# NIFTy-PPL/NIFTy

Hardware: AMD Instinct MI355X
Metric: MGVI iters/sec on 1024^3 RGSpace CorrelatedField, 8 samples; achieved HBM GB/s (higher is better)
Workload: dtype f32

## Files before the change

include/niftyk.h:

```cpp
#ifndef NIFTYK_H
#define NIFTYK_H
#include <stddef.h>
#include <stdint.h>

#ifdef __cplusplus
extern "C" {
#endif

typedef enum {
  NK_OK = 0,
  NK_ERR_INVALID = -1,
  NK_ERR_UNSUPPORTED = -2,
  NK_ERR_RUNTIME = -3,
  NK_ERR_NOMEM = -4
} nk_status;

typedef enum { NK_F32 = 0, NK_F64 = 1 } nk_dtype;

#define NK_HARTLEY_NON_CANONICAL 0
#define NK_HARTLEY_CANONICAL 1

enum { NK_PRO_PLAIN = 0, NK_PRO_AMP = 1, NK_PRO_AMP_JVP = 2, NK_PRO_MUL = 3 };
enum { NK_EPI_AFFINE = 0, NK_EPI_MUL = 1, NK_EPI_VJP = 2, NK_EPI_LIKELIHOOD = 3, NK_EPI_NONLIN = 4 };
enum { NK_LH_GAUSS = 0, NK_LH_POISSON = 1 };
// ... 42 lines not shown
  int io32;
  const void* carry1;
  const void* carry2;
} nk_fuse;

typedef struct nk_plan nk_plan;

const char* nk_last_error(void);
int nk_version(void);

int nk_plan_create(nk_plan** plan, int ndim, const int64_t* shape, int dtype, int64_t batch);
int nk_plan_destroy(nk_plan* plan);
size_t nk_plan_workspace_bytes(const nk_plan* plan);
int nk_hartley(const nk_plan* plan, const void* in, void* out, double scale, int convention, void* workspace,
               void* stream);
int nk_hartley_fused(const nk_plan* plan, const nk_fuse* fuse, int convention, void* workspace, void* stream);
int nk_plan_route(const nk_plan* plan, int route[4]);
int nk_plan_pipe_ok(const nk_plan* plan, int chunks);
int nk_plan_sandwich(const nk_plan* plan);
int nk_hartley_sandwich(const nk_plan* plan, const nk_fuse* fuse, double scale_first, int convention, void* workspace,
                        void* stream);
int nk_hartley_sandwich_pair(const nk_plan* plan, const nk_fuse* fuse_a, const nk_fuse* fuse_b, double scale_first,
                             int convention, void* workspace_a, void* workspace_b, void* stream);
#define NK_MAX_GROUP 4
int nk_hartley_sandwich_group(const nk_plan* plan, const nk_fuse* fuses, int count, double scale_first, int convention,
                              void* const* workspaces, void* stream);
int nk_group_order(int64_t bid, int count, int64_t* member, int64_t* local);
int64_t nk_group_grid_size(int64_t per, int count);
int nk_fftn(const nk_plan* plan, const void* in, void* out, int inverse, double scale, void* workspace,
            void* stream);
int nk_plan_c2c_ok(const nk_plan* plan);
int nk_plan_c2c_lds(const nk_plan* plan, int64_t lds[3]);

int nk_profile_enable(int on);
int nk_profile_collect(double* ms, int64_t* count);

int nk_vdot(int64_t n, const void* a, const void* b, int dtype, double* result, int accumulate, void* stream);

int64_t nk_red_unit(int64_t n, int dtype);
int nk_red_layout(int64_t unit_elems, int k_local, int k_global, int seg_units, int seg_stride, int seg_off,
                  double* units_out);
int nk_red_finish(const double* units, int k_global, int nred, double* result, int accumulate, void* stream);
int nk_sum(int64_t n, const void* a, int dtype, double* result, int accumulate, void* stream);
int nk_stats(int64_t n, const void* a, int dtype, double* result3, void* stream);

enum { NK_OP_ADD = 0, NK_OP_SUB = 1, NK_OP_MUL = 2, NK_OP_DIV = 3 };
// ... 179 lines not shown
```

nifty_amd/_lib.py:

```python
import ctypes
import os

_HERE = os.path.dirname(os.path.abspath(__file__))
LIB_PATH = os.environ.get("NK_LIB_PATH") or os.path.join(_HERE, "csrc", "libniftyk.so")

NK_OK, NK_ERR_INVALID, NK_ERR_UNSUPPORTED, NK_ERR_RUNTIME, NK_ERR_NOMEM = 0, -1, -2, -3, -4
NK_F32, NK_F64 = 0, 1
PRO_PLAIN, PRO_AMP, PRO_AMP_JVP, PRO_MUL = 0, 1, 2, 3
EPI_AFFINE, EPI_MUL, EPI_VJP, EPI_LIKELIHOOD, EPI_NONLIN = 0, 1, 2, 3, 4
LH_GAUSS, LH_POISSON = 0, 1
NL_ID, NL_EXP, NL_SIGMOID = 0, 1, 2
OP_ADD, OP_SUB, OP_MUL, OP_DIV = 0, 1, 2, 3

_vp, _i, _i64, _d, _sz = ctypes.c_void_p, ctypes.c_int, ctypes.c_int64, ctypes.c_double, ctypes.c_size_t


class Fuse(ctypes.Structure):

    _fields_ = [
        ("pro", _i), ("in_", _vp), ("in2", _vp), ("pidx", _vp), ("amp", _vp), ("damp", _vp),
        ("epi", _i), ("out", _vp), ("scale", _d), ("offset", _d), ("mul", _vp), ("mul_scalar", _d),
        ("xi", _vp), ("addend", _vp), ("addend_scale", _d), ("accumulate", _i), ("abar", _vp), ("lh_kind", _i), ("nonlin", _i), ("data", _vp),
        ("icov", _vp), ("icov_scalar", _d), ("out2", _vp), ("value", _vp),
        ("afield", _vp), ("dampT", _vp), ("abar_copies", _i), ("abar_stride", _i64), ("dafield", _vp), ("w8", _vp),
# ... 22 lines not shown
                ("ntiles", _i32 * 3), ("reach", _i32 * 3), ("m", _i64), ("u", _vp), ("perm", _vp), ("bin_start", _vp),
                ("n_items", _i64), ("item", _vp), ("n_split", _i64), ("split_tile", _vp), ("split_slab", _vp), ("corr", _vp)]


class SamplePlan(ctypes.Structure):

    _fields_ = [("ndim", ctypes.c_int32), ("n", _i64 * 3), ("npoints", _i64), ("ncells", _i64), ("nlong", _i64), ("cell", _vp),
                ("frac", _vp), ("perm", _vp), ("cell_start", _vp), ("long_cell", _vp)]


SIGNATURES = {
    "nk_last_error": (ctypes.c_char_p, []),
    "nk_version": (_i, []),
    "nk_plan_create": (_i, [ctypes.POINTER(_vp), _i, ctypes.POINTER(_i64), _i, _i64]),
    "nk_plan_destroy": (_i, [_vp]),
    "nk_plan_workspace_bytes": (_sz, [_vp]),
    "nk_hartley": (_i, [_vp, _vp, _vp, _d, _i, _vp, _vp]),
    "nk_hartley_fused": (_i, [_vp, ctypes.POINTER(Fuse), _i, _vp, _vp]),
    "nk_plan_route": (_i, [_vp, ctypes.POINTER(_i)]),
    "nk_plan_sandwich": (_i, [_vp]),
    "nk_plan_pipe_ok": (_i, [_vp, _i]),
    "nk_hartley_sandwich": (_i, [_vp, ctypes.POINTER(Fuse), _d, _i, _vp, _vp]),
    "nk_hartley_sandwich_pair": (_i, [_vp, ctypes.POINTER(Fuse), ctypes.POINTER(Fuse), _d, _i, _vp, _vp, _vp]),
    "nk_hartley_sandwich_group": (_i, [_vp, ctypes.POINTER(Fuse), _i, _d, _i, _vp, _vp]),
    "nk_group_order": (_i, [_i64, _i, ctypes.POINTER(_i64), ctypes.POINTER(_i64)]),
    "nk_group_grid_size": (_i64, [_i64, _i]),
    "nk_fftn": (_i, [_vp, _vp, _vp, _i, _d, _vp, _vp]),
    "nk_plan_c2c_ok": (_i, [_vp]),
    "nk_plan_c2c_lds": (_i, [_vp, ctypes.POINTER(_i64)]),
    "nk_profile_enable": (_i, [_i]),
    "nk_profile_collect": (_i, [_vp, _vp]),
    "nk_vdot": (_i, [_i64, _vp, _vp, _i, _vp, _i, _vp]),
    "nk_product_field": (_i, [ctypes.POINTER(Product), _i, _vp, _i, _vp]),
    "nk_mirror_combine": (_i, [_i, ctypes.POINTER(_i64), ctypes.POINTER(_i), _i, ctypes.POINTER(_d), _vp, _vp, _d, _d, _i, _vp]),
    "nk_product_marginal_scratch": (_sz, [ctypes.POINTER(Product), _i]),
    "nk_product_marginal": (_i, [ctypes.POINTER(Product), _i, _vp, _vp, _vp, _vp]),
    "nk_red_unit": (_i64, [_i64, _i]),
    "nk_red_layout": (_i, [_i64, _i, _i, _i, _i, _i, _vp]),
    "nk_red_finish": (_i, [_vp, _i, _i, _vp, _i, _vp]),
    "nk_sum": (_i, [_i64, _vp, _i, _vp, _i, _vp]),
    "nk_stats": (_i, [_i64, _vp, _i, _vp, _vp]),
    "nk_binary": (_i, [_i, _i64, _vp, _d, _vp, _d, _vp, _i, _vp]),
    "nk_cplx_muldiv": (_i, [_i64, _vp, _i, _d, _d, _vp, _i, _d, _d, _i, _i, _vp, _i, _vp]),
    "nk_cplx_pointwise": (_i, [_i, _i64, _vp, _vp, _i, _vp]),
    "nk_axpby": (_i, [_i64, _d, _vp, _d, _vp, _vp, _i, _vp]),
    "nk_axpby_sqnorm": (_i, [_i64, _d, _vp, _d, _vp, _vp, _i, _vp, _i, _vp]),
# ... 108 lines not shown
```

nifty_amd/csrc/nk_fft.hip:

```cpp
#include <hip/hip_runtime.h>

#include <algorithm>

#include <cstdio>
#include <cstring>
#include <new>

#include "nk_fft_batch.h"

#include <mutex>
#include <vector>
using ProfScope = NkProfScope;
thread_local const NkBatchCtx* t_batch = nullptr;

template <typename T>
__device__ __forceinline__ void nk_run_stages(C2<T>* lds, int tid, int nthr, const NkLinePlan& lp, const NkTile& tl,
                                              const C2<T>* __restrict__ tw) {
  int L = lp.n;
  for (int s = 0; s < lp.nstage; ++s) {
    const int R = lp.radix[s];
    NK_STAGE_DISPATCH(R, lds, tid, nthr, lp, tl, L, tw, s)
    L /= R;
    __syncthreads();
  }
// ... 1088 lines not shown
  if (count == 1 || !nk_plan_batch_ok(P) || !nk_batch_class_ok(P->hp.g, fuse[0])) {
    for (int m = 0; m < count; ++m) {
      const int rc = P->hp.dtype == NK_F32 ? nk_run_hartley<float>(P, fuse[m], convention, workspace[m], st)
                                           : nk_run_hartley<double>(P, fuse[m], convention, workspace[m], st);
      if (rc != NK_OK) return rc;
    }
    return NK_OK;
  }
  if (P->hp.dtype == NK_F32) return nk_run_hartley_batch<float>(P, fuse, count, convention, workspace, st);
  return nk_run_hartley_batch<double>(P, fuse, count, convention, workspace, st);
}

static bool nk_strided_tile_divides(const nk_plan* P, int n, int64_t inner) {
  return P->hp.dtype == NK_F32 ? nk_fast_strided_ok<float>(n, inner) : nk_fast_strided_ok<double>(n, inner);
}
extern "C" int nk_plan_sandwich(const nk_plan* P) {
  if (!P || !nk_plan_uses_pipeline2(P) || !nk_fast_contig_ok(P->hp.g.h)) return 0;
  const NkGeom& g = P->hp.g;
  const int64_t rs = g.h + (P->hp.dtype == NK_F32 ? nk_pipe3_colpad<float>() : nk_pipe3_colpad<double>());
  if (g.ndim == 3 && !nk_strided_tile_divides(P, g.nm, rs)) return 0;
  return nk_strided_tile_divides(P, g.na, g.ndim == 3 ? (int64_t)g.nm * rs : rs) ? 1 : 0;
}

template <typename T>
static bool nk_contig3_quad_ok(int h) {
  return nk_with_fast_size(h, false, [](auto N) { return (bool)Contig3Tile<T, N()>::QUAD_OK; });
}
extern "C" int nk_plan_pipe_ok(const nk_plan* P, int chunks) {
  if (!nk_plan_sandwich(P) || chunks < 2 || (chunks & 1)) return 0;
  const NkGeom& g = P->hp.g;
  if (g.ndim != 3 || g.batch != 1 || g.na % chunks != 0) return 0;
  if (!nk_knobs().contig_quad || (nk_knobs().xmap & 4)) return 0;
  return (P->hp.dtype == NK_F32 ? nk_contig3_quad_ok<float>(g.h) : nk_contig3_quad_ok<double>(g.h)) ? 1 : 0;
}

template <typename T>
static int nk_run_sandwich(const nk_plan* P, const NkFuse& f, double scale_first, int convention, void* workspace, hipStream_t st,
                           bool with_final = true, NkPipe3* q_out = nullptr, bool with_first = true) {
  const NkHostPlan& hp = P->hp;
  const int sign = convention == NK_HARTLEY_CANONICAL ? -1 : 1;
  const int work_pad = nk_knobs().work_pad;
  const NkPipe3 q = nk_pipe3_setup<T>(hp, sign, work_pad, scale_first * (f.mul_scalar != 0.0 ? f.mul_scalar : 1.0));
  if (q_out) *q_out = q;
  if (nk_pipe3_work_elems(hp.g, nk_pipe3_colpad<T>(), work_pad) * sizeof(C2<T>) > hp.work_bytes)
    return nk_set_error(NK_ERR_RUNTIME, "nk_hartley_sandwich: plan workspace too small");
  if (128 * (q.ss > q.pm.s.inner ? q.ss : q.pm.s.inner) * (int64_t)sizeof(C2<T>) >= ((int64_t)1 << 32))
// ... 366 lines not shown
```

nifty_amd/csrc/nk_fft2.h:

```cpp
#pragma once
#include <type_traits>

#include "nk_fft_phases.h"

template <typename T>
struct TwConst {
  static NK_HD T c(int k) {
    constexpr double v[32] = {1.0,
                              0.99518472667219688624,
                              0.98078528040323044913,
                              0.95694033573220886494,
                              0.92387953251128675613,
                              0.88192126434835502971,
                              0.83146961230254523708,
                              0.77301045336273696081,
                              0.70710678118654752440,
                              0.63439328416364549822,
                              0.55557023301960222474,
                              0.47139673682599764856,
                              0.38268343236508977173,
                              0.29028467725446236764,
                              0.19509032201612826785,
                              0.09801714032956060199,
                              0.0,
// ... 196 lines not shown
#define NK_FINAL_LDS_KB 20
#endif
template <typename T, int NL, int EC = -1, int MINT = 1>
struct FinalTile {
  static constexpr int P = SchedF<T, NL>::P;
  static constexpr int PITCH = ContigLayout<NL, P>::PITCH;
  static constexpr int fit(int tile) {
    return (tile > MINT && (P * tile > 256 || 2 * tile * PITCH * (int)sizeof(T) > NK_FINAL_LDS_KB * 1024)) ? fit(tile / 2) : tile;
  }
  static constexpr int T0 = fit(16);
  static constexpr int TILE = (EC >= 0 && T0 / 2 >= MINT && P * (T0 / 2) >= 64) ? T0 / 2 : T0;
  static constexpr int THREADS = P * TILE;
  static constexpr int LDS_BYTES = 2 * TILE * PITCH * (int)sizeof(T);
};

#ifndef NK_FINAL_SINGLE_2D_KB
#define NK_FINAL_SINGLE_2D_KB 60
#endif
template <typename T, int NL>
constexpr bool nk_final_single_2d() {
  return FinalTile<T, NL, 2, 2>::LDS_BYTES > NK_FINAL_SINGLE_2D_KB * 1024;
}

#ifndef NK_NT_STORE
#define NK_NT_STORE 1
#endif
template <typename T>
NK_HD void nk_store_stream(C2<T>* p, C2<T> v) {
#if !defined(NK_HOST_EMU) && NK_NT_STORE
  typedef T __attribute__((ext_vector_type(2))) V2;
  V2 w;
  w.x = v.x, w.y = v.y;
  __builtin_nontemporal_store(w, reinterpret_cast<V2*>(p));
#else
  *p = v;
#endif
}

template <typename T>
NK_HD void nk_store_stream_s(T* p, T v) {
#if !defined(NK_HOST_EMU) && NK_NT_STORE
  __builtin_nontemporal_store(v, p);
#else
  *p = v;
#endif
}
// ... 508 lines not shown
  c.af = (const T*)f.afield;
  c.c1 = (const T*)f.carry1;
  c.c2 = (const T*)f.carry2;
  c.sc = (T)(f.scale * (EC == 1 ? f.mul_scalar : 1.0));
  c.off = (T)f.offset;
  c.asc = (T)f.addend_scale;
  c.accum = f.accumulate != 0;
  c.dot = EC == 2 && f.value != nullptr && f.addend != nullptr;
  c.keep = f.pipe_chunks < 0;
  c.stash = stash;
  return c;
}

#ifndef NK_FINAL_UNROLL
#define NK_FINAL_UNROLL 1
#endif
#ifndef NK_LH_UNROLL
#define NK_LH_UNROLL 4
#endif
template <typename T>
struct NkVjpOps {
  T x[4], d[4], o[4], p[4], q[4];
};
template <typename T, bool BOTH, int MODE, int STASH = 0>
NK_HD NkVjpOps<T> nk_final_vjp_load(const FinalCt<T>& c, int64_t ok, int64_t om, int k2, int k2m, const T* st = nullptr,
                                    int nkp = 0) {
  NkVjpOps<T> v;
  const bool add = MODE < 0 ? c.addend != nullptr : (MODE & 1) != 0;
  const bool run = MODE < 0 ? c.accum : (MODE & 2) != 0;
  const bool k1 = MODE < 0 ? c.c1 != nullptr : (MODE & 4) != 0;
  const bool k2nd = MODE < 0 ? c.c2 != nullptr : (MODE & 8) != 0;
  const int64_t rowb[4] = {ok, om, ok, om};
  const uint32_t colb[4] = {(uint32_t)k2, (uint32_t)k2m, (uint32_t)k2m, (uint32_t)k2};
#pragma unroll
  for (int i = 0; i < 4; ++i) {
    const bool on = BOTH || i < 2;
    if constexpr (STASH == 3)
      v.p[i] = on ? st[i * nkp] : (T)0;
    else
      v.p[i] = (on && k1) ? (c.c1 + rowb[i])[colb[i]] : (T)0;
    v.q[i] = (on && k2nd) ? (c.c2 + rowb[i])[colb[i]] : (T)0;
    if constexpr ((NK_NT_LOAD & 8) != 0) {
      v.x[i] = on ? nk_ld_stream((c.xi + rowb[i]) + colb[i]) : (T)0;
      v.d[i] = (on && add) ? nk_ld_stream((c.addend + rowb[i]) + colb[i]) : (T)0;
      if constexpr (STASH == 2)
        v.o[i] = on ? st[i * nkp] : (T)0;
      else
        v.o[i] = (on && run) ? nk_ld_stream((c.out + rowb[i]) + colb[i]) : (T)0;
    } else {
      v.x[i] = on ? (c.xi + rowb[i])[colb[i]] : (T)0;
      v.d[i] = (on && add) ? (c.addend + rowb[i])[colb[i]] : (T)0;
      if constexpr (STASH == 2)
        v.o[i] = on ? st[i * nkp] : (T)0;
      else
        v.o[i] = (on && run) ? (c.out + rowb[i])[colb[i]] : (T)0;
    }
  }
  return v;
}
template <typename T, bool BOTH, int MODE, int STASH = 0>
NK_HD double nk_final_vjp_apply(const FinalCt<T>& c, const NkVjpOps<T>& v, int64_t ok, int64_t om, bool self, T v0, T v1,
                                T v2, T v3, int k2, int k2m, T a, double& acc, T* st = nullptr, int nkp = 0) {
  const T t[4] = {v0 * c.sc, v1 * c.sc, v2 * c.sc, v3 * c.sc};
  const bool k1 = STASH == 3 || (MODE < 0 ? c.c1 != nullptr : (MODE & 4) != 0);
  const bool k2nd = MODE < 0 ? c.c2 != nullptr : (MODE & 8) != 0;
  T r[4];
#pragma unroll
  for (int i = 0; i < 4; ++i) {
    r[i] = nk_settle(a * t[i]);
    r[i] = nk_settle(nk_fma(c.asc, v.d[i], r[i]));
    if (k1) r[i] = v.p[i] + r[i];
    if (k2nd) r[i] = v.q[i] + r[i];
    r[i] = v.o[i] + r[i];
  }
  if (c.dot) {
    double e = (double)v.d[0] * (double)r[0];
    if (BOTH) e += (double)v.d[2] * (double)r[2];
    if (!self) e += (double)v.d[1] * (double)r[1] + (BOTH ? (double)v.d[3] * (double)r[3] : 0.0);
    acc += e;
  }
  T* outk = c.out + ok;
  T* outm = c.out + om;
  auto put = [&](T* p, T val, int image) {
    if constexpr (STASH == 1)
      st[image * nkp] = val;
    else if (c.keep)
      *p = val;
    else
      nk_store_stream_s(p, val);
  };
  put(outk + (uint32_t)k2, r[0], 0);
  if (BOTH) put(outk + (uint32_t)k2m, r[2], 2);
  double s = (double)v.x[0] * (double)t[0];
  if (BOTH) s += (double)v.x[2] * (double)t[2];
  if (!self) {
    put(outm + (uint32_t)k2m, r[1], 1);
    s += (double)v.x[1] * (double)t[1];
    if (BOTH) {
      put(outm + (uint32_t)k2, r[3], 3);
      s += (double)v.x[3] * (double)t[3];
    }
  }
  return s;
}

template <typename T, int EC, bool BOTH, int MODE = -1>
NK_HD double nk_final_slot(const NkFuse& f, const FinalCt<T>& c, int64_t ok, int64_t om, bool self, T sg, T fx, T fy, T gx,
// ... 29 lines not shown
      if (BOTH) nk_store_stream_s(outk + k2m, (T)(v2 * c.sc * m2));
      if (!self) {
        nk_store_stream_s(outm + k2m, (T)(v1 * c.sc * m1));
        if (BOTH) nk_store_stream_s(outm + k2, (T)(v3 * c.sc * m3));
      }
    } else {
      nk_store_stream_s(outk + k2, (T)(v0 * c.sc));
      if (BOTH) nk_store_stream_s(outk + k2m, (T)(v2 * c.sc));
      if (!self) {
        nk_store_stream_s(outm + k2m, (T)(v1 * c.sc));
        if (BOTH) nk_store_stream_s(outm + k2, (T)(v3 * c.sc));
      }
    }
    return 0.0;
  } else {
    static_assert(EC != 2, "the scatter epilogue runs through nk_final_vjp_load / nk_final_vjp_apply");
    return 0.0;
  }
}

template <typename T, int NL, int NH, bool BOTH, int MODE, int U, int STASH = 0>
NK_HD void nk_final_vjp_coeffs(const NkFuse& f, const FinalCt<T>& c, const FinalGroup<NH>& gp, const T* pre, const T* pim, T sg,
                               const int (&k2s)[U], int n_on, int hv, const T* afline, double* w8line, double& acc,
                               float& wmax) {
  constexpr int NKP = NL / 2 + 1;
  NkVjpOps<T> ops[U][NH];
  T a[U];
#pragma unroll
  for (int u = 0; u < U; ++u) {
    const int k2 = k2s[u], k2m = (NL - k2) & (NL - 1);
    a[u] = afline[k2];
#pragma unroll
    for (int h = 0; h < NH; ++h)
      if (MODE >= 0 || gp.mlo[h]) {
        if constexpr (STASH >= 2)
          ops[u][h] = nk_final_vjp_load<T, BOTH, MODE, STASH>(c, gp.okh[h], gp.omh[h], k2, k2m, c.stash + h * 4 * NKP + k2, NKP);
        else
          ops[u][h] = nk_final_vjp_load<T, BOTH, MODE>(c, gp.okh[h], gp.omh[h], k2, k2m);
      }
  }
#pragma unroll
  for (int u = 0; u < U; ++u) {
    if (u >= n_on) break;
    const int k2 = k2s[u], k2m = (NL - k2) & (NL - 1);
    const int d1 = k2 + (k2 >> 5), d2 = k2m + (k2m >> 5);
    double ssum = 0.0;
#pragma unroll
    for (int h = 0; h < NH; ++h) {
      if (MODE < 0 && !gp.mlo[h]) continue;
      const T fx = pre[gp.base[h] + d1], fy = pim[gp.base[h] + d1];
      const T gx = pre[gp.base[h] + d2], gy = pim[gp.base[h] + d2];
      if constexpr (STASH != 0)
        ssum += nk_final_vjp_apply<T, BOTH, MODE, STASH>(c, ops[u][h], gp.okh[h], gp.omh[h], gp.mlo[h] == 1, fx + sg * fy,
                                                         fx - sg * fy, gx + sg * gy, gx - sg * gy, k2, k2m, a[u], acc,
                                                         c.stash + h * 4 * NKP + k2, NKP);
      else
        ssum += nk_final_vjp_apply<T, BOTH, MODE>(c, ops[u][h], gp.okh[h], gp.omh[h], gp.mlo[h] == 1, fx + sg * fy, fx - sg * fy,
                                                  gx + sg * gy, gx - sg * gy, k2, k2m, a[u], acc);
    }
    if (w8line) {
      w8line[k2] = ssum;
      wmax = nk_wmax_join(wmax, nk_abs_up(ssum));
    } else {
      NK_VJP_SCATTER(f, f.pidx[gp.okh[hv] + k2], ssum);
    }
  }
}

template <typename T, int NL, int NH, bool BOTH, int MODE, int U, typename TD = T>
NK_HD void nk_final_lh_coeffs(const NkFuse& f, const FinalGroup<NH>& gp, const T* pre, const T* pim, T sg, const int (&k2s)[U],
                              int n_on, double& acc) {
  constexpr int MASK = BOTH ? 15 : 3;
  typename NkLhData<TD, MODE>::type d[U][NH][4];
#pragma unroll
  for (int u = 0; u < U; ++u) {
    const int k2 = k2s[u], k2m = (NL - k2) & (NL - 1);
#pragma unroll
    for (int h = 0; h < NH; ++h) {
// ... 3 lines not shown
  }
#pragma unroll
  for (int u = 0; u < U; ++u) {
    if (u >= n_on) break;
    const int k2 = k2s[u], k2m = (NL - k2) & (NL - 1);
    const int d1 = k2 + (k2 >> 5), d2 = k2m + (k2m >> 5);
    double ssum = 0.0;
#pragma unroll
    for (int h = 0; h < NH; ++h) {
      const T fx = pre[gp.base[h] + d1], fy = pim[gp.base[h] + d1];
      const T gx = pre[gp.base[h] + d2], gy = pim[gp.base[h] + d2];
      const int64_t o4[4] = {gp.okh[h] + k2, gp.omh[h] + k2m, gp.okh[h] + k2m, gp.omh[h] + k2};
      const T v4[4] = {fx + sg * fy, fx - sg * fy, gx + sg * gy, gx - sg * gy};
      double e = 0.0;
      nk_lh4_apply<T, MODE, MASK, TD>(f, o4, v4, d[u][h], e);
      ssum += e;
    }
    acc += ssum;
  }
}

template <typename T, int NL, int NH, int EC, bool BOTH, int MODE = -1, int STASH = 0>
NK_HD void nk_final_coeff(const NkFuse& f, const FinalCt<T>& c, const FinalGroup<NH>& gp, const T* pre, const T* pim, T sg,
                          int k2, int hv, const T* afline, double* w8line, double& acc, float& wmax) {
  if constexpr (EC == 2) {
    const int one[1] = {k2};
    nk_final_vjp_coeffs<T, NL, NH, BOTH, MODE, 1, STASH>(f, c, gp, pre, pim, sg, one, 1, hv, afline, w8line, acc, wmax);
  } else {
    const int k2m = (NL - k2) & (NL - 1);
    const int d1 = k2 + (k2 >> 5), d2 = k2m + (k2m >> 5);
    double ssum = 0.0;
#pragma unroll
    for (int h = 0; h < NH; ++h) {
      if (MODE <= 0 && !gp.mlo[h]) continue;
      const T fx = pre[gp.base[h] + d1], fy = pim[gp.base[h] + d1];
      const T gx = pre[gp.base[h] + d2], gy = pim[gp.base[h] + d2];
      ssum += nk_final_slot<T, EC, BOTH, MODE>(f, c, gp.okh[h], gp.omh[h], gp.mlo[h] == 1, sg, fx, fy, gx, gy, k2, k2m, (T)0,
                                               acc);
    }
    if constexpr (nk_ec_lh<EC>()) acc += ssum;
  }
}

struct NkPassF {
  NkGeom g;
  int A, M;
  int tiles_per_a;
  int blo;
  int64_t ss;
  int64_t rs;
// ... 153 lines not shown
    const int lane = tid - u * tps;
    constexpr int NH = COUPLES ? 2 : 1;
    FinalGroup<NH> gp;
    int any = 0;
    double* w8line = nullptr;
    const int b0g = couples ? bt0 * (TILE / 2) + u : bt0 * TILE + u;
    if (f.w8 && f.epi == NK_EPI_VJP)
      w8line = f.w8 + ((bat * (A / 2 + 1) + a) * (int64_t)(M / 2 + 1) + b0g) * (NL / 2 + 1);
#pragma unroll
    for (int h = 0; h < NH; ++h) {
      const int t = couples ? 2 * u + h : u;
      int b, bm;
      bool active, self;
      line_of(t, b, bm, active, self);
      if (h == 1 && !couples) active = false;
      gp.okh[h] = (((bat * A + a) * M + b)) * (int64_t)NL;
      gp.omh[h] = (((bat * A + am) * M + bm)) * (int64_t)NL;
      gp.base[h] = LY::addr(t, 0);
      gp.mlo[h] = active ? (self ? 1 : 3) : 0;
      any |= gp.mlo[h];
    }
    if constexpr (EC >= 0) {
      if (any) {
        const FinalCt<T> c = nk_final_ct<T, EC>(f, STASH != 0 ? stash + u * (NH * 4 * (NL / 2 + 1)) : nullptr);
        int hv = 0;
#pragma unroll
        for (int h = NH - 1; h >= 0; --h)
          if (gp.mlo[h]) hv = h;
        const T* afline = nullptr;
        if constexpr (EC == 2)
          afline = f.field_octant ? c.af + ((int64_t)a * (M / 2 + 1) + b0g) * (NL / 2 + 1) : c.af + gp.okh[hv];
        auto coefficients = [&](auto mode_c) {
          constexpr int MODE = decltype(mode_c)::value;
          if (lane < 2)
            nk_final_coeff<T, NL, NH, EC, false, MODE, STASH>(f, c, gp, pre, pim, sg, lane ? NL / 2 : 0, hv, afline, w8line, acc, wmax);
          if constexpr (nk_ec_lh<EC>() && MODE > 0) {
            constexpr int U = sizeof(T) == 8 ? (NK_LH_UNROLL + 1) / 2 : NK_LH_UNROLL;
            for (int k2 = 1 + lane; k2 < NL / 2; k2 += U * tps) {
              int ks[U], n_on = 0;
#pragma unroll
              for (int u = 0; u < U; ++u) {
                const int k = k2 + u * tps;
                const bool on = k < NL / 2;
                ks[u] = on ? k : k2;
                n_on += on;
              }
              nk_final_lh_coeffs<T, NL, NH, true, MODE, U, typename NkLhIo<T, EC>::type>(f, gp, pre, pim, sg, ks, n_on, acc);
            }
          } else if constexpr (EC == 2 && MODE >= 0 && NK_FINAL_UNROLL > 1) {
            constexpr int U = NK_FINAL_UNROLL;
            for (int k2 = 1 + lane; k2 < NL / 2; k2 += U * tps) {
              int ks[U], n_on = 0;
#pragma unroll
              for (int u = 0; u < U; ++u) {
                const int k = k2 + u * tps;
                const bool on = k < NL / 2;
                ks[u] = on ? k : k2;
                n_on += on;
              }
              nk_final_vjp_coeffs<T, NL, NH, true, MODE, U, STASH>(f, c, gp, pre, pim, sg, ks, n_on, hv, afline, w8line, acc, wmax);
            }
          } else {
            for (int k2 = 1 + lane; k2 < NL / 2; k2 += tps)
              nk_final_coeff<T, NL, NH, EC, true, MODE, STASH>(f, c, gp, pre, pim, sg, k2, hv, afline, w8line, acc, wmax);
          }
        };
        if constexpr (EC == 2) {
          bool full = true;
#pragma unroll
          for (int h = 0; h < NH; ++h) full = full && gp.mlo[h] != 0;
          switch (full ? (c.addend ? 1 : 0) | (c.accum ? 2 : 0) | (c.c1 ? 4 : 0) | (c.c2 ? 8 : 0) : -1) {
            case 0: coefficients(std::integral_constant<int, 0>{}); break;
            case 1: coefficients(std::integral_constant<int, 1>{}); break;
            case 2: coefficients(std::integral_constant<int, 2>{}); break;
            case 3: coefficients(std::integral_constant<int, 3>{}); break;
            case 6: coefficients(std::integral_constant<int, 6>{}); break;
            case 14: coefficients(std::integral_constant<int, 14>{}); break;
            default: coefficients(std::integral_constant<int, -1>{}); break;
          }
        } else if constexpr (nk_ec_lh<EC>()) {
          bool regular = true;
#pragma unroll
          for (int h = 0; h < NH; ++h) regular = regular && gp.mlo[h] == 3;
          const bool gauss = f.lh_kind == NK_LH_GAUSS;
          switch (regular && !(gauss && f.icov) ? (gauss ? 1 : 2) : -1) {
            case 1: coefficients(std::integral_constant<int, 1>{}); break;
            case 2: coefficients(std::integral_constant<int, 2>{}); break;
            default: coefficients(std::integral_constant<int, -1>{}); break;
          }
        } else {
          coefficients(std::integral_constant<int, -1>{});
        }
      }
    } else if (any) {
// ... 152 lines not shown
```

nifty_amd/csrc/nk_fft_batch.h:

```cpp
#pragma once
#include "nk_plan.h"
#include "nk_fft2.h"
#include "nk_util.h"

#ifndef NK_S0_WAVES
#define NK_S0_WAVES 1
#endif
#ifndef NK_PAIR_HAND_LDS_KB
#define NK_PAIR_HAND_LDS_KB 64
#endif
#ifndef NK_S1_TWO_WG
#define NK_S1_TWO_WG 0
#endif

template <typename T, bool COUPLES, int EC, int THREADS>
constexpr int nk_final_waves() {
  return THREADS > 256 ? 1 : (sizeof(T) == 8 && (COUPLES || EC == 2)) ? 2 : ((!COUPLES && sizeof(T) == 4 && (EC == 0 || EC == 1)) ? 4 : 3);
}

__device__ __forceinline__ void nk_flush_energy(const NkFuse& f, double acc, void* lds_raw) {
  if ((f.epi != NK_EPI_LIKELIHOOD && f.epi != NK_EPI_VJP) || f.value == nullptr) return;
  for (int off = 32; off > 0; off >>= 1) acc += __shfl_down(acc, off, 64);
  const int lane = threadIdx.x & 63, wave = threadIdx.x >> 6;
  const int nw = (blockDim.x + 63) >> 6;
// ... 52 lines not shown
static bool nk_batch_class_ok(const NkGeom& g, const nk_fuse& f) {
  if (nk_knobs().ec_generic || g.na < 512 || g.nl < 512) return false;
  const bool pro_ok = f.pro == NK_PRO_PLAIN || f.pro == NK_PRO_MUL ||
                      (f.field_octant && !f.io32 && (f.pro == NK_PRO_AMP || f.pro == NK_PRO_AMP_JVP));
  const bool epi_ok = f.epi == NK_EPI_MUL || (f.epi == NK_EPI_LIKELIHOOD && !f.io32) || f.epi == NK_EPI_NONLIN ||
                      (f.epi == NK_EPI_VJP && f.afield);
  return pro_ok && epi_ok;
}


template <typename T, int N, int PC>
int nk_twin_launch_strided(const NkPassS& ps, int64_t blocks, const C2<T>* tw, int xmap, hipStream_t st);
template <typename T, int NL, bool COUPLES, int EC>
int nk_twin_launch_final(const NkPassF& pf, int64_t blocks, const C2<T>* tw, int xmap, hipStream_t st);

template <typename T>
int nk_tl_first_axis(const NkPassS& s1, int n1, int n2, const NkFuse& f, const C2<T>* tw_n1, const C2<T>* tw_n2, const C2<T>* tw_full,
                     C2<T>* work, hipStream_t st);

template <typename T, int NL>
int nk_launch_final_pair(NkPassF pf, const NkFuse& fa, const NkFuse& fb, const C2<T>* tw, const C2<T>* worka, const C2<T>* workb,
                         hipStream_t st);

NK_HD void nk_group_decode(int64_t bid, int count, int64_t& member, int64_t& local) {
  const int64_t span = 8 * (int64_t)count;
  const int64_t g = bid / span, w = bid % span;
  member = w / 8;
  local = 8 * g + w % 8;
}
static inline int64_t nk_group_grid(int64_t per, int count) { return (per + 7) / 8 * 8 * count; }
struct NkGroupFuse {
  NkFuse f[NK_MAX_GROUP];
};
struct NkGroupWork {
  void* work[NK_MAX_GROUP];
};

#ifndef NK_QUAD_MAXW_F64_5
#define NK_QUAD_MAXW_F64_5 4
#endif
#ifndef NK_QUAD_MAXW_F64_8
#define NK_QUAD_MAXW_F64_8 8
#endif
#ifndef NK_QUAD_MAXW_F32_5
#define NK_QUAD_MAXW_F32_5 8
#endif
// ... 18 lines not shown
```

nifty_amd/csrc/nk_fft_p.hip:

```cpp
#include <hip/hip_runtime.h>

#include "nk_fft_batch.h"

#ifndef NK_PAIR_HAND_BUILD
#define NK_PAIR_HAND_BUILD 0
#endif
template <typename T, int NL>
struct PairTile {
  using CT = FinalTile<T, NL, 2, 2>;
  static constexpr int STASH_BYTES = CT::TILE * 4 * (NL / 2 + 1) * (int)sizeof(T);
  static constexpr int LDS_HAND = CT::LDS_BYTES + STASH_BYTES;
  static constexpr bool HAND_OK = NK_PAIR_HAND_BUILD != 0 && LDS_HAND <= NK_PAIR_HAND_LDS_KB * 1024;
};

#ifndef NK_PAIR_HAND_WAVES
#define NK_PAIR_HAND_WAVES 3
#endif
template <typename T, int NL, int HAND>
__global__ void __launch_bounds__((FinalTile<T, NL, 2, 2>::THREADS),
                                  (HAND ? (FinalTile<T, NL, 2, 2>::THREADS > 256 ? 1 : NK_PAIR_HAND_WAVES)
                                        : nk_final_waves<T, true, 2, FinalTile<T, NL, 2, 2>::THREADS>()))
    k2_final2(NkPassF p, NkFuse fa, NkFuse fb, const C2<T>* __restrict__ tw, const C2<T>* __restrict__ worka,
              const C2<T>* __restrict__ workb) {
  extern __shared__ __align__(16) unsigned char smem[];
  using CT = FinalTile<T, NL, 2, 2>;
  DeviceExec<T, SchedF<T, NL>::E> ex;
  const int64_t blk = (int64_t)blockIdx.x;
  T* stash = HAND ? (T*)(smem + CT::LDS_BYTES) : nullptr;
  fa.pipe_chunks = -1;
  {
    double acc = 0.0;
    float wmax = 0.0f;
    nk_final_body<T, NL, CT::TILE, true, 2, 1, HAND ? 1 : 0>(ex, p, fa, blk, (T*)smem, tw, worka, &acc, &wmax, stash);
    nk_flush_energy(fa, acc, smem);
    nk_flush_wmax(fa, wmax);
  }
  __syncthreads();
  {
    double acc = 0.0;
    float wmax = 0.0f;
    nk_final_body<T, NL, CT::TILE, true, 2, 1, HAND>(ex, p, fb, blk, (T*)smem, tw, workb, &acc, &wmax, stash);
    nk_flush_energy(fb, acc, smem);
    nk_flush_wmax(fb, wmax);
  }
}

template <typename T, int NL, int HAND>
static int nk_launch_final_pair_h(NkPassF pf, const NkFuse& fa, const NkFuse& fb, const C2<T>* tw, const C2<T>* worka,
                                  const C2<T>* workb, hipStream_t st) {
  using CT = FinalTile<T, NL, 2, 2>;
  const int LDS = HAND ? PairTile<T, NL>::LDS_HAND : CT::LDS_BYTES + nk_knobs().pair_pad_lds;
  pf.tiles_per_a = (pf.A > 1 && CT::TILE >= 2) ? (pf.M / 2 + 1 + CT::TILE / 2 - 1) / (CT::TILE / 2) : (pf.M + CT::TILE - 1) / CT::TILE;
  pf.blk0 = 0;
  const int64_t blocks = (int64_t)pf.g.batch * (pf.A / 2 + 1) * pf.tiles_per_a;
  const int64_t waves = blocks * ((CT::THREADS + 63) / 64);
  if ((fa.value_slots > 0 && waves > fa.value_slots) || (fb.value_slots > 0 && waves > fb.value_slots))
    return nk_set_error(NK_ERR_RUNTIME, "final pass: more wavefronts than reduction slots (nk_value_slot_count)");
  return nk_launch<k2_final2<T, NL, HAND>>("k2_final2", dim3((unsigned)blocks), dim3(CT::THREADS), LDS, st, pf, fa, fb, tw, worka, workb);
}

template <typename T, int NL>
int nk_launch_final_pair(NkPassF pf, const NkFuse& fa, const NkFuse& fb, const C2<T>* tw, const C2<T>* worka, const C2<T>* workb,
                         hipStream_t st) {
  if constexpr (PairTile<T, NL>::HAND_OK) {
    if (nk_knobs().pair_hand && pf.A > 1) {
      if (fa.out == fb.out && fb.accumulate) return nk_launch_final_pair_h<T, NL, 2>(pf, fa, fb, tw, worka, workb, st);
      if (fb.carry1 == fa.out && fb.out != fa.out) return nk_launch_final_pair_h<T, NL, 3>(pf, fa, fb, tw, worka, workb, st);
    }
  }
  return nk_launch_final_pair_h<T, NL, 0>(pf, fa, fb, tw, worka, workb, st);
}

#define NK_CASE(NN)                                                                                                             \
  template int nk_launch_final_pair<float, NN>(NkPassF, const NkFuse&, const NkFuse&, const C2<float>*, const C2<float>*,        \
                                               const C2<float>*, hipStream_t);                                                  \
  template int nk_launch_final_pair<double, NN>(NkPassF, const NkFuse&, const NkFuse&, const C2<double>*, const C2<double>*,     \
                                                const C2<double>*, hipStream_t);
NK_FAST_SIZES(NK_CASE)
#undef NK_CASE
```

nifty_amd/csrc/nk_plan.h:

```cpp
#pragma once
#include <cmath>
#include <cstdlib>
#include <vector>

#include "nk_fft_phases.h"

static inline NkLinePlan nk_make_line_plan(int n) {
  NkLinePlan lp{};
  lp.n = n;
  lp.nstage = 0;
  int rem = n;
  while (rem > 1) {
    int R;
    if (rem % 8 == 0) R = (rem == 16) ? 4 : 8;
    else if (rem % 4 == 0) R = 4;
    else if (rem % 2 == 0) R = 2;
    else if (rem % 3 == 0) R = 3;
    else if (rem % 5 == 0) R = 5;
    else if (rem % 7 == 0) R = 7;
    else {
      lp.nstage = -1;
      return lp;
    }
    if (lp.nstage == NK_MAX_STAGES) {
// ... 3 lines not shown
    lp.radix[lp.nstage++] = R;
    rem /= R;
  }
  int span = n;
  for (int s = 0; s < lp.nstage; ++s) {
    span /= lp.radix[s];
    lp.span[s] = span;
    lp.dradix[s] = nk_make_div(lp.radix[s]);
    lp.dspan[s] = nk_make_div(span);
    lp.dnbf[s] = nk_make_div(n / lp.radix[s]);
  }
  return lp;
}
static inline bool nk_factorable(int64_t n) { return n >= 1 && n < ((int64_t)1 << 30) && nk_make_line_plan((int)n).nstage >= 0; }

static inline int nk_env_int(const char* name, int dflt) {
  const char* v = getenv(name);
  return v ? atoi(v) : dflt;
}

#ifndef NK_XMAP_DEFAULT
#define NK_XMAP_DEFAULT 9
#endif
struct NkKnobs {
  int fast = 1;
  int pipeline = 2;
  int xmap = NK_XMAP_DEFAULT;
  int work_blo = 0;
  int work_pad = 2080;
  int contig_quad = 1;
  int ec_generic = 0;
  int two_level = 1;
  int skip_final = 0;
  int mid_wg_per_cu = 0;
  int pair_hand = 0;
  int pair_pad_lds = 0;
  int group = 1;
  int tile_divides = 0;
};
static inline NkKnobs nk_read_knobs() {
  NkKnobs k;
  k.fast = nk_env_int("NK_FAST", k.fast);
  k.pipeline = nk_env_int("NK_PIPELINE", k.pipeline);
  k.xmap = nk_env_int("NK_XMAP", k.xmap);
  k.work_blo = nk_env_int("NK_WORK_BLO", k.work_blo);
  k.work_pad = nk_env_int("NK_WORK_PAD", k.work_pad);
  k.contig_quad = nk_env_int("NK_CONTIG_QUAD", k.contig_quad);
  k.ec_generic = nk_env_int("NK_EC_GENERIC", k.ec_generic);
  k.two_level = nk_env_int("NK_TWO_LEVEL", k.two_level);
  k.skip_final = nk_env_int("NK_SKIP_FINAL", k.skip_final);
  k.mid_wg_per_cu = nk_env_int("NK_MID_WG_PER_CU", k.mid_wg_per_cu);
  k.pair_hand = nk_env_int("NK_PAIR_HAND", k.pair_hand);
  k.pair_pad_lds = nk_env_int("NK_PAIR_PAD_LDS", k.pair_pad_lds);
  k.group = nk_env_int("NK_GROUP", k.group);
  k.tile_divides = nk_env_int("NK_TILE_DIVIDES", k.tile_divides);
  return k;
}
inline NkKnobs nk_knobs() {
// ... 172 lines not shown
```

Before: 0.2199.

## Hand over paired final-pass VJP values through registers instead of LDS stash

Adds a register-resident hand-over (HAND bit 4) to the paired final Hartley kernel, so the first fused epilogue stashes its per-coefficient outputs in a per-thread register array that the second epilogue reads back directly. This avoids both re-reading the output/carry arrays from HBM and allocating an LDS stash. It is enabled by default through a new pair_hand default of 2. The cost is higher register pressure in the kernel, which may reduce occupancy or cause spills, and it relies on each thread visiting the same coefficients in both halves.

```diff
diff --git a/include/niftyk.h b/include/niftyk.h
--- a/include/niftyk.h
+++ b/include/niftyk.h
@@ -88,6 +88,7 @@
                         void* stream);
 int nk_hartley_sandwich_pair(const nk_plan* plan, const nk_fuse* fuse_a, const nk_fuse* fuse_b, double scale_first,
                              int convention, void* workspace_a, void* workspace_b, void* stream);
+int nk_plan_pair_hand(const nk_plan* plan);
 #define NK_MAX_GROUP 4
 int nk_hartley_sandwich_group(const nk_plan* plan, const nk_fuse* fuses, int count, double scale_first, int convention,
                               void* const* workspaces, void* stream);
diff --git a/nifty_amd/_lib.py b/nifty_amd/_lib.py
--- a/nifty_amd/_lib.py
+++ b/nifty_amd/_lib.py
@@ -68,6 +68,7 @@
     "nk_plan_pipe_ok": (_i, [_vp, _i]),
     "nk_hartley_sandwich": (_i, [_vp, ctypes.POINTER(Fuse), _d, _i, _vp, _vp]),
     "nk_hartley_sandwich_pair": (_i, [_vp, ctypes.POINTER(Fuse), ctypes.POINTER(Fuse), _d, _i, _vp, _vp, _vp]),
+    "nk_plan_pair_hand": (_i, [_vp]),
     "nk_hartley_sandwich_group": (_i, [_vp, ctypes.POINTER(Fuse), _i, _d, _i, _vp, _vp]),
     "nk_group_order": (_i, [_i64, _i, ctypes.POINTER(_i64), ctypes.POINTER(_i64)]),
     "nk_group_grid_size": (_i64, [_i64, _i]),
diff --git a/nifty_amd/csrc/nk_fft.hip b/nifty_amd/csrc/nk_fft.hip
--- a/nifty_amd/csrc/nk_fft.hip
+++ b/nifty_amd/csrc/nk_fft.hip
@@ -1134,6 +1134,13 @@
   return nk_strided_tile_divides(P, g.na, g.ndim == 3 ? (int64_t)g.nm * rs : rs) ? 1 : 0;
 }
 
+extern "C" int nk_plan_pair_hand(const nk_plan* P) {
+  if (!nk_plan_sandwich(P) || P->hp.g.ndim != 3) return -1;
+  const int nl = P->hp.g.nl;
+  if (P->hp.dtype == NK_F32) return nk_with_fast_size(nl, -1, [](auto N) { return nk_pair_hand_form<float, N()>(); });
+  return nk_with_fast_size(nl, -1, [](auto N) { return nk_pair_hand_form<double, N()>(); });
+}
+
 template <typename T>
 static bool nk_contig3_quad_ok(int h) {
   return nk_with_fast_size(h, false, [](auto N) { return (bool)Contig3Tile<T, N()>::QUAD_OK; });
diff --git a/nifty_amd/csrc/nk_fft2.h b/nifty_amd/csrc/nk_fft2.h
--- a/nifty_amd/csrc/nk_fft2.h
+++ b/nifty_amd/csrc/nk_fft2.h
@@ -242,6 +242,22 @@
   return FinalTile<T, NL, 2, 2>::LDS_BYTES > NK_FINAL_SINGLE_2D_KB * 1024;
 }
 
+template <typename T, int NL>
+struct FinalHand {
+  static constexpr int TPS = 2 * SchedF<T, NL>::P;
+  static constexpr int TRIPS = (NL / 2 - 1 + TPS - 1) / TPS;
+  static constexpr int N = (TRIPS + 1) * 2 * 4;
+};
+template <typename T, int NL>
+NK_HD T* nk_hand_of(T* hand, int tid) {
+#ifdef NK_HOST_EMU
+  return hand + (size_t)tid * FinalHand<T, NL>::N;
+#else
+  (void)tid;
+  return hand;
+#endif
+}
+
 #ifndef NK_NT_STORE
 #define NK_NT_STORE 1
 #endif
@@ -796,20 +812,24 @@
 struct NkVjpOps {
   T x[4], d[4], o[4], p[4], q[4];
 };
+template <int STASH>
+constexpr bool nk_stash_no_carry() {
+  return STASH == 5;
+}
 template <typename T, bool BOTH, int MODE, int STASH = 0>
 NK_HD NkVjpOps<T> nk_final_vjp_load(const FinalCt<T>& c, int64_t ok, int64_t om, int k2, int k2m, const T* st = nullptr,
                                     int nkp = 0) {
   NkVjpOps<T> v;
   const bool add = MODE < 0 ? c.addend != nullptr : (MODE & 1) != 0;
   const bool run = MODE < 0 ? c.accum : (MODE & 2) != 0;
-  const bool k1 = MODE < 0 ? c.c1 != nullptr : (MODE & 4) != 0;
-  const bool k2nd = MODE < 0 ? c.c2 != nullptr : (MODE & 8) != 0;
+  const bool k1 = !nk_stash_no_carry<STASH>() && (MODE < 0 ? c.c1 != nullptr : (MODE & 4) != 0);
+  const bool k2nd = !nk_stash_no_carry<STASH>() && (MODE < 0 ? c.c2 != nullptr : (MODE & 8) != 0);
   const int64_t rowb[4] = {ok, om, ok, om};
   const uint32_t colb[4] = {(uint32_t)k2, (uint32_t)k2m, (uint32_t)k2m, (uint32_t)k2};
 #pragma unroll
   for (int i = 0; i < 4; ++i) {
     const bool on = BOTH || i < 2;
-    if constexpr (STASH == 3)
+    if constexpr ((STASH & 3) == 3)
       v.p[i] = on ? st[i * nkp] : (T)0;
     else
       v.p[i] = (on && k1) ? (c.c1 + rowb[i])[colb[i]] : (T)0;
@@ -817,14 +837,14 @@
     if constexpr ((NK_NT_LOAD & 8) != 0) {
       v.x[i] = on ? nk_ld_stream((c.xi + rowb[i]) + colb[i]) : (T)0;
       v.d[i] = (on && add) ? nk_ld_stream((c.addend + rowb[i]) + colb[i]) : (T)0;
-      if constexpr (STASH == 2)
+      if constexpr ((STASH & 3) == 2)
         v.o[i] = on ? st[i * nkp] : (T)0;
       else
         v.o[i] = (on && run) ? nk_ld_stream((c.out + rowb[i]) + colb[i]) : (T)0;
     } else {
       v.x[i] = on ? (c.xi + rowb[i])[colb[i]] : (T)0;
       v.d[i] = (on && add) ? (c.addend + rowb[i])[colb[i]] : (T)0;
-      if constexpr (STASH == 2)
+      if constexpr ((STASH & 3) == 2)
         v.o[i] = on ? st[i * nkp] : (T)0;
       else
         v.o[i] = (on && run) ? (c.out + rowb[i])[colb[i]] : (T)0;
@@ -836,8 +856,8 @@
 NK_HD double nk_final_vjp_apply(const FinalCt<T>& c, const NkVjpOps<T>& v, int64_t ok, int64_t om, bool self, T v0, T v1,
                                 T v2, T v3, int k2, int k2m, T a, double& acc, T* st = nullptr, int nkp = 0) {
   const T t[4] = {v0 * c.sc, v1 * c.sc, v2 * c.sc, v3 * c.sc};
-  const bool k1 = STASH == 3 || (MODE < 0 ? c.c1 != nullptr : (MODE & 4) != 0);
-  const bool k2nd = MODE < 0 ? c.c2 != nullptr : (MODE & 8) != 0;
+  const bool k1 = (STASH & 3) == 3 || (!nk_stash_no_carry<STASH>() && (MODE < 0 ? c.c1 != nullptr : (MODE & 4) != 0));
+  const bool k2nd = !nk_stash_no_carry<STASH>() && (MODE < 0 ? c.c2 != nullptr : (MODE & 8) != 0);
   T r[4];
 #pragma unroll
   for (int i = 0; i < 4; ++i) {
@@ -856,7 +876,7 @@
   T* outk = c.out + ok;
   T* outm = c.out + om;
   auto put = [&](T* p, T val, int image) {
-    if constexpr (STASH == 1)
+    if constexpr ((STASH & 3) == 1)
       st[image * nkp] = val;
     else if (c.keep)
       *p = val;
@@ -932,8 +952,10 @@
 template <typename T, int NL, int NH, bool BOTH, int MODE, int U, int STASH = 0>
 NK_HD void nk_final_vjp_coeffs(const NkFuse& f, const FinalCt<T>& c, const FinalGroup<NH>& gp, const T* pre, const T* pim, T sg,
                                const int (&k2s)[U], int n_on, int hv, const T* afline, double* w8line, double& acc,
-                               float& wmax) {
+                               float& wmax, int slot = 0) {
   constexpr int NKP = NL / 2 + 1;
+  constexpr int SKP = (STASH & 4) ? 1 : NKP;
+  auto stash_at = [&](int u, int h, int k2) { return (STASH & 4) ? c.stash + ((slot + u) * NH + h) * 4 : c.stash + h * 4 * NKP + k2; };
   NkVjpOps<T> ops[U][NH];
   T a[U];
 #pragma unroll
@@ -943,8 +965,8 @@
 #pragma unroll
     for (int h = 0; h < NH; ++h)
       if (MODE >= 0 || gp.mlo[h]) {
-        if constexpr (STASH >= 2)
-          ops[u][h] = nk_final_vjp_load<T, BOTH, MODE, STASH>(c, gp.okh[h], gp.omh[h], k2, k2m, c.stash + h * 4 * NKP + k2, NKP);
+        if constexpr ((STASH & 3) >= 2)
+          ops[u][h] = nk_final_vjp_load<T, BOTH, MODE, STASH>(c, gp.okh[h], gp.omh[h], k2, k2m, stash_at(u, h, k2), SKP);
         else
           ops[u][h] = nk_final_vjp_load<T, BOTH, MODE>(c, gp.okh[h], gp.omh[h], k2, k2m);
       }
@@ -963,7 +985,7 @@
       if constexpr (STASH != 0)
         ssum += nk_final_vjp_apply<T, BOTH, MODE, STASH>(c, ops[u][h], gp.okh[h], gp.omh[h], gp.mlo[h] == 1, fx + sg * fy,
                                                          fx - sg * fy, gx + sg * gy, gx - sg * gy, k2, k2m, a[u], acc,
-                                                         c.stash + h * 4 * NKP + k2, NKP);
+                                                         stash_at(u, h, k2), SKP);
       else
         ssum += nk_final_vjp_apply<T, BOTH, MODE>(c, ops[u][h], gp.okh[h], gp.omh[h], gp.mlo[h] == 1, fx + sg * fy, fx - sg * fy,
                                                   gx + sg * gy, gx - sg * gy, k2, k2m, a[u], acc);
@@ -1013,10 +1035,10 @@
 
 template <typename T, int NL, int NH, int EC, bool BOTH, int MODE = -1, int STASH = 0>
 NK_HD void nk_final_coeff(const NkFuse& f, const FinalCt<T>& c, const FinalGroup<NH>& gp, const T* pre, const T* pim, T sg,
-                          int k2, int hv, const T* afline, double* w8line, double& acc, float& wmax) {
+                          int k2, int hv, const T* afline, double* w8line, double& acc, float& wmax, int slot = 0) {
   if constexpr (EC == 2) {
     const int one[1] = {k2};
-    nk_final_vjp_coeffs<T, NL, NH, BOTH, MODE, 1, STASH>(f, c, gp, pre, pim, sg, one, 1, hv, afline, w8line, acc, wmax);
+    nk_final_vjp_coeffs<T, NL, NH, BOTH, MODE, 1, STASH>(f, c, gp, pre, pim, sg, one, 1, hv, afline, w8line, acc, wmax, slot);
   } else {
     const int k2m = (NL - k2) & (NL - 1);
     const int d1 = k2 + (k2 >> 5), d2 = k2m + (k2m >> 5);
@@ -1216,7 +1238,8 @@
     }
     if constexpr (EC >= 0) {
       if (any) {
-        const FinalCt<T> c = nk_final_ct<T, EC>(f, STASH != 0 ? stash + u * (NH * 4 * (NL / 2 + 1)) : nullptr);
+        static_assert((STASH & 4) == 0 || (COUPLES && EC == 2 && TILE >= 2), "the register hand-over serves the VJP epilogue on line couples");
+        const FinalCt<T> c = nk_final_ct<T, EC>(f, (STASH & 4) ? nk_hand_of<T, NL>(stash, tid) : STASH != 0 ? stash + u * (NH * 4 * (NL / 2 + 1)) : nullptr);
         int hv = 0;
 #pragma unroll
         for (int h = NH - 1; h >= 0; --h)
@@ -1226,6 +1249,17 @@
           afline = f.field_octant ? c.af + ((int64_t)a * (M / 2 + 1) + b0g) * (NL / 2 + 1) : c.af + gp.okh[hv];
         auto coefficients = [&](auto mode_c) {
           constexpr int MODE = decltype(mode_c)::value;
+          if constexpr ((STASH & 4) != 0) {
+            using FH = FinalHand<T, NL>;
+            if (lane < 2)
+              nk_final_coeff<T, NL, NH, EC, false, MODE, STASH>(f, c, gp, pre, pim, sg, lane ? NL / 2 : 0, hv, afline, w8line, acc, wmax, FH::TRIPS);
+#pragma unroll
+            for (int j = 0; j < FH::TRIPS; ++j) {
+              const int k2 = 1 + lane + j * FH::TPS;
+              if (k2 < NL / 2) nk_final_coeff<T, NL, NH, EC, true, MODE, STASH>(f, c, gp, pre, pim, sg, k2, hv, afline, w8line, acc, wmax, j);
+            }
+            return;
+          }
           if (lane < 2)
             nk_final_coeff<T, NL, NH, EC, false, MODE, STASH>(f, c, gp, pre, pim, sg, lane ? NL / 2 : 0, hv, afline, w8line, acc, wmax);
           if constexpr (nk_ec_lh<EC>() && MODE > 0) {
@@ -1263,7 +1297,7 @@
           bool full = true;
 #pragma unroll
           for (int h = 0; h < NH; ++h) full = full && gp.mlo[h] != 0;
-          switch (full ? (c.addend ? 1 : 0) | (c.accum ? 2 : 0) | (c.c1 ? 4 : 0) | (c.c2 ? 8 : 0) : -1) {
+          switch (full ? (c.addend ? 1 : 0) | (c.accum ? 2 : 0) | (c.c1 && !nk_stash_no_carry<STASH>() ? 4 : 0) | (c.c2 && !nk_stash_no_carry<STASH>() ? 8 : 0) : -1) {
             case 0: coefficients(std::integral_constant<int, 0>{}); break;
             case 1: coefficients(std::integral_constant<int, 1>{}); break;
             case 2: coefficients(std::integral_constant<int, 2>{}); break;
diff --git a/nifty_amd/csrc/nk_fft_batch.h b/nifty_amd/csrc/nk_fft_batch.h
--- a/nifty_amd/csrc/nk_fft_batch.h
+++ b/nifty_amd/csrc/nk_fft_batch.h
@@ -98,6 +98,9 @@
 int nk_launch_final_pair(NkPassF pf, const NkFuse& fa, const NkFuse& fb, const C2<T>* tw, const C2<T>* worka, const C2<T>* workb,
                          hipStream_t st);
 
+template <typename T, int NL>
+int nk_pair_hand_form();
+
 NK_HD void nk_group_decode(int64_t bid, int count, int64_t& member, int64_t& local) {
   const int64_t span = 8 * (int64_t)count;
   const int64_t g = bid / span, w = bid % span;
diff --git a/nifty_amd/csrc/nk_fft_p.hip b/nifty_amd/csrc/nk_fft_p.hip
--- a/nifty_amd/csrc/nk_fft_p.hip
+++ b/nifty_amd/csrc/nk_fft_p.hip
@@ -5,38 +5,70 @@
 #ifndef NK_PAIR_HAND_BUILD
 #define NK_PAIR_HAND_BUILD 0
 #endif
+#ifndef NK_PAIR_REGS_BUILD
+#define NK_PAIR_REGS_BUILD 1
+#endif
 template <typename T, int NL>
 struct PairTile {
   using CT = FinalTile<T, NL, 2, 2>;
   static constexpr int STASH_BYTES = CT::TILE * 4 * (NL / 2 + 1) * (int)sizeof(T);
   static constexpr int LDS_HAND = CT::LDS_BYTES + STASH_BYTES;
   static constexpr bool HAND_OK = NK_PAIR_HAND_BUILD != 0 && LDS_HAND <= NK_PAIR_HAND_LDS_KB * 1024;
+  static constexpr bool REGS_OK = NK_PAIR_REGS_BUILD != 0;
 };
 
 #ifndef NK_PAIR_HAND_WAVES
 #define NK_PAIR_HAND_WAVES 3
 #endif
+template <typename T, int E>
+struct DeviceExecAt {
+  PassRegs<T, E>& regs;
+  int tid;
+  template <typename F>
+  __device__ __forceinline__ void phase(F f) {
+    f(tid, regs);
+    __syncthreads();
+  }
+  template <typename F>
+  __device__ __forceinline__ void last_phase(F f) {
+    f(tid, regs);
+  }
+};
+
 template <typename T, int NL, int HAND>
 __global__ void __launch_bounds__((FinalTile<T, NL, 2, 2>::THREADS),
-                                  (HAND ? (FinalTile<T, NL, 2, 2>::THREADS > 256 ? 1 : NK_PAIR_HAND_WAVES)
-                                        : nk_final_waves<T, true, 2, FinalTile<T, NL, 2, 2>::THREADS>()))
+                                  (HAND == 2 || HAND == 3 ? (FinalTile<T, NL, 2, 2>::THREADS > 256 ? 1 : NK_PAIR_HAND_WAVES)
+                                                          : nk_final_waves<T, true, 2, FinalTile<T, NL, 2, 2>::THREADS>()))
     k2_final2(NkPassF p, NkFuse fa, NkFuse fb, const C2<T>* __restrict__ tw, const C2<T>* __restrict__ worka,
               const C2<T>* __restrict__ workb) {
   extern __shared__ __align__(16) unsigned char smem[];
   using CT = FinalTile<T, NL, 2, 2>;
   DeviceExec<T, SchedF<T, NL>::E> ex;
   const int64_t blk = (int64_t)blockIdx.x;
-  T* stash = HAND ? (T*)(smem + CT::LDS_BYTES) : nullptr;
+  constexpr bool REGS = (HAND & 4) != 0;
+  T hand[REGS ? FinalHand<T, NL>::N : 1];
+  T* stash = REGS ? hand : HAND ? (T*)(smem + CT::LDS_BYTES) : nullptr;
   fa.pipe_chunks = -1;
   {
     double acc = 0.0;
     float wmax = 0.0f;
-    nk_final_body<T, NL, CT::TILE, true, 2, 1, HAND ? 1 : 0>(ex, p, fa, blk, (T*)smem, tw, worka, &acc, &wmax, stash);
+    nk_final_body<T, NL, CT::TILE, true, 2, 1, HAND ? (HAND & 4) | 1 : 0>(ex, p, fa, blk, (T*)smem, tw, worka, &acc, &wmax, stash);
     nk_flush_energy(fa, acc, smem);
     nk_flush_wmax(fa, wmax);
   }
   __syncthreads();
-  {
+  if constexpr (REGS) {
+    int64_t blkb = blk;
+    int tidb = (int)threadIdx.x;
+    asm volatile("" : "+s"(blkb));
+    asm volatile("" : "+v"(tidb));
+    DeviceExecAt<T, SchedF<T, NL>::E> exb{ex.regs, tidb};
+    double acc = 0.0;
+    float wmax = 0.0f;
+    nk_final_body<T, NL, CT::TILE, true, 2, 1, HAND>(exb, p, fb, blkb, (T*)smem, tw, workb, &acc, &wmax, stash);
+    nk_flush_energy(fb, acc, smem);
+    nk_flush_wmax(fb, wmax);
+  } else {
     double acc = 0.0;
     float wmax = 0.0f;
     nk_final_body<T, NL, CT::TILE, true, 2, 1, HAND>(ex, p, fb, blk, (T*)smem, tw, workb, &acc, &wmax, stash);
@@ -49,7 +81,7 @@
 static int nk_launch_final_pair_h(NkPassF pf, const NkFuse& fa, const NkFuse& fb, const C2<T>* tw, const C2<T>* worka,
                                   const C2<T>* workb, hipStream_t st) {
   using CT = FinalTile<T, NL, 2, 2>;
-  const int LDS = HAND ? PairTile<T, NL>::LDS_HAND : CT::LDS_BYTES + nk_knobs().pair_pad_lds;
+  const int LDS = (HAND & 4) ? CT::LDS_BYTES : HAND ? PairTile<T, NL>::LDS_HAND : CT::LDS_BYTES + nk_knobs().pair_pad_lds;
   pf.tiles_per_a = (pf.A > 1 && CT::TILE >= 2) ? (pf.M / 2 + 1 + CT::TILE / 2 - 1) / (CT::TILE / 2) : (pf.M + CT::TILE - 1) / CT::TILE;
   pf.blk0 = 0;
   const int64_t blocks = (int64_t)pf.g.batch * (pf.A / 2 + 1) * pf.tiles_per_a;
@@ -62,8 +94,14 @@
 template <typename T, int NL>
 int nk_launch_final_pair(NkPassF pf, const NkFuse& fa, const NkFuse& fb, const C2<T>* tw, const C2<T>* worka, const C2<T>* workb,
                          hipStream_t st) {
+  if constexpr (PairTile<T, NL>::REGS_OK) {
+    if (nk_knobs().pair_hand == 2 && pf.A > 1 && !fa.carry1 && !fa.carry2) {
+      if (fa.out == fb.out && fb.accumulate) return nk_launch_final_pair_h<T, NL, 6>(pf, fa, fb, tw, worka, workb, st);
+      if (fb.carry1 == fa.out && fb.out != fa.out) return nk_launch_final_pair_h<T, NL, 7>(pf, fa, fb, tw, worka, workb, st);
+    }
+  }
   if constexpr (PairTile<T, NL>::HAND_OK) {
-    if (nk_knobs().pair_hand && pf.A > 1) {
+    if (nk_knobs().pair_hand == 1 && pf.A > 1) {
       if (fa.out == fb.out && fb.accumulate) return nk_launch_final_pair_h<T, NL, 2>(pf, fa, fb, tw, worka, workb, st);
       if (fb.carry1 == fa.out && fb.out != fa.out) return nk_launch_final_pair_h<T, NL, 3>(pf, fa, fb, tw, worka, workb, st);
     }
@@ -71,7 +109,16 @@
   return nk_launch_final_pair_h<T, NL, 0>(pf, fa, fb, tw, worka, workb, st);
 }
 
+template <typename T, int NL>
+int nk_pair_hand_form() {
+  if (PairTile<T, NL>::REGS_OK && nk_knobs().pair_hand == 2) return 2;
+  if (PairTile<T, NL>::HAND_OK && nk_knobs().pair_hand == 1) return 1;
+  return 0;
+}
+
 #define NK_CASE(NN)                                                                                                             \
+  template int nk_pair_hand_form<float, NN>();                                                                                  \
+  template int nk_pair_hand_form<double, NN>();                                                                                 \
   template int nk_launch_final_pair<float, NN>(NkPassF, const NkFuse&, const NkFuse&, const C2<float>*, const C2<float>*,        \
                                                const C2<float>*, hipStream_t);                                                  \
   template int nk_launch_final_pair<double, NN>(NkPassF, const NkFuse&, const NkFuse&, const C2<double>*, const C2<double>*,     \
diff --git a/nifty_amd/csrc/nk_plan.h b/nifty_amd/csrc/nk_plan.h
--- a/nifty_amd/csrc/nk_plan.h
+++ b/nifty_amd/csrc/nk_plan.h
@@ -49,6 +49,9 @@
 #ifndef NK_XMAP_DEFAULT
 #define NK_XMAP_DEFAULT 9
 #endif
+#ifndef NK_PAIR_HAND_DEFAULT
+#define NK_PAIR_HAND_DEFAULT 2
+#endif
 struct NkKnobs {
   int fast = 1;
   int pipeline = 2;
@@ -60,7 +63,7 @@
   int two_level = 1;
   int skip_final = 0;
   int mid_wg_per_cu = 0;
-  int pair_hand = 0;
+  int pair_hand = NK_PAIR_HAND_DEFAULT;
   int pair_pad_lds = 0;
   int group = 1;
   int tile_divides = 0;
```

Measured after the change: 0.2210, median of 6. About the same (+0.5%).
